# unanan/UNet_Nested4Tiny_Objects_Keypoints

Measured on AMD Instinct MI355X. Metric: images/sec (train step) UNet++ L=4 256x256, higher is better.
Workload: dtype f32

## Files before the change

include/unetpp_hip.h:

```cpp
#ifndef UNETPP_HIP_H
#define UNETPP_HIP_H

#include <stdint.h>

#ifdef __cplusplus
extern "C" {
#endif

#define UNETPP_ABI_VERSION 12
#define UNETPP_MAX_VIEWS 8

#define UNETPP_OK 0
#define UNETPP_EINVAL (-1)
#define UNETPP_ELAUNCH (-2)

typedef struct unetpp_view {
  float* ptr;
  int32_t C, c_off, c_len;
  int32_t Hs, Ws;
  int32_t sy, sx, oy, ox;
  const float* scale;
  const float* shift;
  const float* gate;
  int32_t relu;
// ... 135 lines not shown
                             int32_t W, int32_t C, float* dy, void* stream);

int64_t unetpp_bn_frozen_bwd_blocks(int64_t pixels, int32_t C);
int unetpp_bn_frozen_bwd(const float* d_act, const float* y, const float* scale, const float* shift,
                         const float* mean, const float* invstd, const float* d_pooled, const uint8_t* pool_idx,
                         int32_t N, int32_t H, int32_t W, int32_t C, float* dy, float* partial, void* stream);

int unetpp_head_fwd(const float* x, const float* weight, const float* bias, int32_t N, int32_t H, int32_t W,
                    int32_t C, int32_t n_cls, float p_drop, uint64_t seed, const uint8_t* mask, const uint64_t* seed_dev,
                    float* out_nchw, void* stream);
int64_t unetpp_head_bwd_blocks(int64_t pixels);
int unetpp_head_bwd(const float* d_out_nchw, const float* out_nchw, const float* x, const float* weight,
                    int32_t N, int32_t H, int32_t W, int32_t C, int32_t n_cls, float p_drop, uint64_t seed,
                    const uint8_t* mask, const uint64_t* seed_dev, float* dx, int32_t accumulate, int32_t gate_x, float* partial,
                    void* stream);
int unetpp_sum_partials(const float* partial, int64_t n_blocks, int64_t len, float* out, void* stream);

int unetpp_bilinear2x_fwd(const float* x, int32_t N, int32_t H, int32_t W, int32_t C, float* y, void* stream);
int unetpp_bilinear2x_bwd(const float* dy, int32_t N, int32_t H, int32_t W, int32_t C, float* dx, int32_t accumulate,
                          void* stream);

int64_t unetpp_focal_bce_blocks(int64_t n);
int unetpp_focal_bce(const float* pred, const float* target, int64_t n, int64_t rows, float gamma, float* grad,
                     float* partial, float* loss, void* stream);
#define UNETPP_MAX_HEADS 8
typedef struct unetpp_focal_heads {
  const float* pred[UNETPP_MAX_HEADS];
  float* grad[UNETPP_MAX_HEADS];
  int32_t n_heads, reserved;
} unetpp_focal_heads;
// ... 100 lines not shown
```

unet_nested4tiny_objects_keypoints_amd/_lib.py:

```python
from __future__ import annotations

import ctypes as C
import os
import subprocess

_PKG_DIR = os.path.dirname(os.path.abspath(__file__))
_REPO = os.path.dirname(_PKG_DIR)
LIB_PATH = os.environ.get("UNETPP_LIB", os.path.join(_PKG_DIR, "libunetpp_hip.so"))
CSRC = os.path.join(_PKG_DIR, "csrc")
INCLUDE = os.path.join(_REPO, "include")
SOURCES = ("gemm_pix.hip", "gemm_fast.hip", "gemm_pw.hip", "gemm_pw_bf16.hip", "gemm_wino.hip", "gemm_bf16.hip", "gemm_bf16_dma.hip", "wgrad_bf16.hip", "pointwise_bf16.hip", "keypoints.hip", "weight_image.hip", "wgrad.hip", "wgrad_fast.hip", "wgrad_dma.hip", "wgrad_pw.hip", "wgrad_wino.hip", "first_layer.hip", "pointwise.hip", "caller.hip", "optim.hip", "validate.hip")
HEADERS = ("common.h", "gemm_units.h", "wgrad_reduce.h", "lds_asm.h", "bf16_common.h", "dropout.h", "bn_fused.h",
           "wino_experiments.h", "dma_experiments.h", "heads_mean.h")
MAX_VIEWS = 8
ABI_VERSION = 12
EXTRA_FLAGS = {"gemm_wino.hip": ("-fno-slp-vectorize",), "wgrad_wino.hip": ("-fno-slp-vectorize",)}
GEMM_DIRECT = 1
GEMM_BF16 = 2


class View(C.Structure):
    _fields_ = [
        ("ptr", C.c_void_p),
        ("C", C.c_int32), ("c_off", C.c_int32), ("c_len", C.c_int32),
# ... 120 lines not shown
    "unetpp_pack_weight": (C.c_int, [_P, _P, _I32, _I32, _I32, _I64, _I64, _I64, _I64, _I64, _I64, _I32, _P]),
    "unetpp_bn_finalize": (C.c_int, [_P, _I64, _I32, _I64, _P, _P, _F, _F, _P, _P, _P, _P, _P, _P, _P]),
    "unetpp_bn_eval_coeffs": (C.c_int, [_P, _P, _P, _P, _F, _I32, _P, _P, _P]),
    "unetpp_affine_relu_pool": (C.c_int, [_P, _P, _P, _I32, _I32, _I32, _I32, _I32, _P, _P, _P, _P]),
    "unetpp_maxpool_bwd": (C.c_int, [_P, _P, _I32, _I32, _I32, _I32, _P, _P]),
    "unetpp_bn_bwd_blocks": (_I64, [_I64, _I32]),
    "unetpp_bn_bwd_reduce": (C.c_int, [_P, _P, _P, _P, _P, _P, _I64, _I32, _P, _P]),
    "unetpp_bn_bwd_finalize": (C.c_int, [_P, _I64, _I32, _P, _P, _P]),
    "unetpp_bn_bwd_apply": (C.c_int, [_P, _P, _P, _P, _P, _P, _P, _P, _P, _I64, _I32, _P, _P]),
    "unetpp_bn_bwd_pool_ok": (C.c_int, [_I32, _I32, _I32, _I32]),
    "unetpp_bn_bwd_reduce_pool": (C.c_int, [_P, _P, _P, _P, _P, _P, _P, _P, _I32, _I32, _I32, _I32, _P, _P]),
    "unetpp_bn_bwd_apply_pool": (C.c_int, [_P, _P, _P, _P, _P, _P, _P, _P, _P, _P, _P, _I32, _I32, _I32, _I32, _P, _P]),
    "unetpp_head_fwd": (C.c_int, [_P, _P, _P, _I32, _I32, _I32, _I32, _I32, _F, _U64, _P, _P, _P, _P]),
    "unetpp_head_bwd_blocks": (_I64, [_I64]),
    "unetpp_head_bwd": (C.c_int, [_P, _P, _P, _P, _I32, _I32, _I32, _I32, _I32, _F, _U64, _P, _P, _P, _I32, _I32, _P, _P]),
    "unetpp_sum_partials": (C.c_int, [_P, _I64, _I64, _P, _P]),
    "unetpp_focal_bce_blocks": (_I64, [_I64]),
    "unetpp_focal_bce": (C.c_int, [_P, _P, _I64, _I64, _F, _P, _P, _P, _P]),
    "unetpp_focal_bce_heads": (C.c_int, [C.POINTER(FocalHeads), _P, _I64, _I64, _F, _P, _P, _P]),
    "unetpp_heads_mean_fwd": (C.c_int, [C.POINTER(HeadsMean), _I32, _I32, _I32, _I32, _I32, _P, _P]),
    "unetpp_heads_mean_fwd_bf16": (C.c_int, [C.POINTER(HeadsMean), _I32, _I32, _I32, _I32, _I32, _P, _P]),
    "unetpp_bn_eval_coeffs_stats": (C.c_int, [_P, _P, _P, _P, _F, _I32, _P, _P, _P, _P, _P]),
    "unetpp_bn_frozen_bwd_blocks": (_I64, [_I64, _I32]),
    "unetpp_bn_frozen_bwd": (C.c_int, [_P, _P, _P, _P, _P, _P, _P, _P, _I32, _I32, _I32, _I32, _P, _P, _P]),
    "unetpp_bn_frozen_bwd_blocks_bf16": (_I64, [_I64, _I32]),
    "unetpp_bn_frozen_bwd_bf16": (C.c_int, [_P, _P, _P, _P, _P, _P, _P, _P, _I32, _I32, _I32, _I32, _P, _P, _P]),
    "unetpp_copy_jobs": (C.c_int, [_P, _I32, _I64, _P]),
    "unetpp_heatmap_workspace_bytes": (_I64, [_I32, _I32, _I32]),
    "unetpp_create_heatmap": (C.c_int, [_P, _I32, _I32, _I32, _I32, _F, _P, _P, _P]),
    "unetpp_bilinear2x_fwd": (C.c_int, [_P, _I32, _I32, _I32, _I32, _P, _P]),
# ... 111 lines not shown
```

unet_nested4tiny_objects_keypoints_amd/csrc/caller.hip:

```cpp
#include "common.h"

namespace unetpp {
namespace {

constexpr int kLossThreads = 256;
constexpr int kLossPerThread = 8;

__device__ __forceinline__ float focal_thread(const float* __restrict__ pred, float* __restrict__ grad,
                                              const float (&t)[kLossPerThread / 4][4], long base, long n, float gamma,
                                              float inv_rows, float scale) {
  const bool cube = gamma == 3.f;
  float sum = 0.f;
#pragma unroll
  for (int h = 0; h < kLossPerThread / 4; ++h) {
    const long i = base + 4 * h;
    if (i >= n) break;
    float p[4], g[4];
    const bool vec = (i + 4 <= n);
    if (vec) {
      const f32x4 pv = *reinterpret_cast<const f32x4*>(pred + i);
#pragma unroll
      for (int e = 0; e < 4; ++e) p[e] = pv[e];
    } else {
#pragma unroll
      for (int e = 0; e < 4; ++e) p[e] = (i + e < n) ? pred[i + e] : 0.f;
    }
#pragma unroll
    for (int e = 0; e < 4; ++e) {
      const float d = p[e] - t[h][e];
      const float err = (1.f - fabsf(d)) + 1e-20f;
      const float u = 1.f - err;
      const float lg = logf(err);
      const float ug1 = cube ? u * u : powf(u, gamma - 1.f);
      const float ug = ug1 * u;
      const float le = -ug * lg;
      const float dl_de = gamma * ug1 * lg - ug / err;
      const float sgn = (d > 0.f) ? 1.f : ((d < 0.f) ? -1.f : 0.f);
      g[e] = (-dl_de * sgn * inv_rows) * scale;
      if (i + e < n) sum += le;
    }
    if (grad != nullptr) {
      if (vec) {
        *reinterpret_cast<f32x4*>(grad + i) = f32x4{g[0], g[1], g[2], g[3]};
      } else {
#pragma unroll
        for (int e = 0; e < 4; ++e)
          if (i + e < n) grad[i + e] = g[e];
      }
    }
  }
  return sum;
}

// ... 231 lines not shown
```

unet_nested4tiny_objects_keypoints_amd/csrc/common.h:

```cpp
#pragma once
#include <hip/hip_runtime.h>
#include <stdint.h>

#include "unetpp_hip.h"

typedef float f32x16 __attribute__((ext_vector_type(16)));
typedef float f32x4 __attribute__((ext_vector_type(4)));

namespace unetpp {

constexpr int kBlockPixels = 256;
constexpr int kThreads = 256;
constexpr int kMaxHaloPixels = 340;

struct TileGeom {
  int log2tw, tiles_x, tiles_y;
};

inline TileGeom tile_geom(int H, int W) {
  int l = 3;
  while ((1 << l) < W && l < 5) ++l;
  TileGeom g;
  g.log2tw = l;
  const int TW = 1 << l, TH = kBlockPixels >> l;
// ... 7 lines not shown
  static_assert(OFF == 1 || OFF == 2 || OFF == 4 || OFF == 8 || OFF == 16, "xor_lane: 1, 2, 4, 8 or 16");
  const int i = __builtin_bit_cast(int, v);
  int r;
  if constexpr (OFF == 1) r = __builtin_amdgcn_mov_dpp(i, 0xB1, 0xF, 0xF, true);
  else if constexpr (OFF == 2) r = __builtin_amdgcn_mov_dpp(i, 0x4E, 0xF, 0xF, true);
  else r = __builtin_amdgcn_ds_swizzle(i, 0x1F | (OFF << 10));
  return __builtin_bit_cast(float, r);
}

__device__ __forceinline__ float row16_sum(float v) {
  v += xor_lane<1>(v);
  v += xor_lane<2>(v);
  v += __builtin_bit_cast(float, __builtin_amdgcn_mov_dpp(__builtin_bit_cast(int, v), 0x141, 0xF, 0xF, true));
  v += __builtin_bit_cast(float, __builtin_amdgcn_mov_dpp(__builtin_bit_cast(int, v), 0x140, 0xF, 0xF, true));
  return v;
}

inline int finish_log2_groups(int n_split) {
  int l = 0;
  while ((1 << l) < n_split && l < 4) ++l;
  return l;
}

inline bool view_ok(const unetpp_view& v, bool need_ptr = true) {
  if (need_ptr && v.ptr == nullptr) return false;
  if (v.C <= 0 || v.c_len <= 0 || v.c_off < 0 || v.c_off + v.c_len > v.C) return false;
  if (v.Hs <= 0 || v.Ws <= 0 || v.sy <= 0 || v.sx <= 0 || v.oy < 0 || v.ox < 0) return false;
  if ((v.scale == nullptr) != (v.shift == nullptr)) return false;
  return true;
}
// ... 127 lines not shown
```

unet_nested4tiny_objects_keypoints_amd/csrc/pointwise.hip:

```cpp
#include "common.h"
#include "lds_asm.h"
#include "dropout.h"
#include "heads_mean.h"

namespace unetpp {
namespace {

template <int VEC>
struct Pack;
template <>
struct Pack<4> {
  using T = f32x4;
};
template <>
struct Pack<1> {
  using T = float;
};
template <int VEC>
__device__ __forceinline__ float& lane_of(typename Pack<VEC>::T& v, int i) {
  if constexpr (VEC == 4)
    return reinterpret_cast<float*>(&v)[i];
  else
    return v;
}
// ... 1067 lines not shown
        f32x4 old = {0.f, 0.f, 0.f, 0.f};
        if (accumulate) old = *reinterpret_cast<const f32x4*>(dx + off);
#pragma unroll
        for (int q = 0; q < 4; ++q) {
          float v = sacc[q] * ms[q] + old[q];
          if (gate_x) v = (xv[q] > 0.f) ? v : 0.f;
          sacc[q] = v;
        }
        *reinterpret_cast<f32x4*>(dx + off) = sacc;
      }
      float* xd = &xs[pl * XS + 4 * gq];
#pragma unroll
      for (int q = 0; q < 4; ++q) xd[q] = xv[q] * ms[q];
    }
    __syncthreads();
#pragma unroll
    for (int q = 0; q < kMaxPairs; ++q) {
      if (pair0 + q * 128 < NW) {
        const int k = pair_k[q], c = pair_c[q];
        float sum = 0.f;
#pragma unroll 4
        for (int pl = 32 * half; pl < 32 * half + 32; ++pl) sum += dl[pl * kHeadMaxCls + k] * xs[pl * XS + c];
        wacc[q] += sum;
      }
    }
    if (tid < n_cls) {
      float sum = 0.f;
      for (int pl = 0; pl < 64; ++pl) sum += dl[pl * kHeadMaxCls + tid];
      bacc += sum;
    }
// ... 667 lines not shown
  if ((C & 3) == 0 && aligned16(x) && aligned16(dx)) {
    const size_t lds = (64 * (C + 1) + 64 * kHeadMaxCls + kHeadMaxCls * C + 2 * n_cls * C) * sizeof(float);
    note_kernel("head_bwd_vec");
    hipLaunchKernelGGL(head_bwd_vec_kernel, dim3(static_cast<unsigned>(unetpp_head_bwd_blocks(pixels))), dim3(kThreads),
                       lds, ST(stream), d_out_nchw, out_nchw, x, weight, pixels, H * W, C, n_cls, 1.0f / (1.0f - p_drop),
                       keep_threshold(p_drop), seed, mask, seed_dev, use_drop, dx, accumulate, gate_x, partial);
    return launch_status();
  }
  note_kernel("head_bwd");
  hipLaunchKernelGGL(head_bwd_kernel, dim3(static_cast<unsigned>(unetpp_head_bwd_blocks(pixels))), dim3(kThreads), 0,
                     ST(stream), d_out_nchw, out_nchw, x, weight, pixels, H * W, C, n_cls, 1.0f / (1.0f - p_drop),
                     keep_threshold(p_drop), seed, mask, seed_dev, use_drop, dx, accumulate, gate_x, partial);
  return launch_status();
}

extern "C" int unetpp_sum_partials(const float* partial, int64_t n_blocks, int64_t len, float* out, void* stream) {
  if (!partial || !out || n_blocks < 1 || len < 1) return UNETPP_EINVAL;
  hipLaunchKernelGGL(sum_partials_kernel, dim3(static_cast<unsigned>((len + 15) / 16)), dim3(1024), 0, ST(stream),
                     partial, n_blocks, len, out);
  return launch_status();
}

extern "C" int unetpp_bilinear2x_fwd(const float* x, int32_t N, int32_t H, int32_t W, int32_t C, float* y, void* stream) {
  if (!x || !y || N < 1 || H < 1 || W < 1 || C < 1) return UNETPP_EINVAL;
  const long items = static_cast<long>(N) * 4 * H * W * C;
  note_kernel("bilinear2x_fwd");
  hipLaunchKernelGGL(bilinear2x_fwd_kernel, dim3(grid_for(items)), dim3(kThreads), 0, ST(stream), x, N, H, W, C, y);
  return launch_status();
}

// ... 30 lines not shown
```

unet_nested4tiny_objects_keypoints_amd/engine.py:

```python
from __future__ import annotations

import os

from typing import Dict, List, Optional, Tuple

import torch

from . import ops
from .ops import V


USE_PACK_PLAN = os.environ.get("UNETPP_NO_PACK_PLAN") is None
USE_GROUPED_DGRAD = os.environ.get("UNETPP_NO_GROUPED_DGRAD") is None
USE_PLAN_COPIES = os.environ.get("UNETPP_NO_PLAN_COPIES") is None
_A1_MATERIALIZE_BYTES = int(float(os.environ.get("UNETPP_BF16_A1_MAX_MB", "80")) * (1 << 20))
_A1_MATERIALIZE_BYTES_F32 = int(float(os.environ.get("UNETPP_F32_A1_MAX_MB", "80")) * (1 << 20))


def _empty(n, like):
    return torch.empty(n, dtype=torch.float32, device=like.device)


def _packed(w, t, k, n, dstr, sstr, flip=False):
    dst = _empty(t * k * n, w)
# ... 198 lines not shown


def check_head(depth: int, head) -> int:
    if head is None:
        return depth - 1
    if isinstance(head, bool) or not isinstance(head, int) or not 1 <= head <= depth - 1:
        raise ValueError("head must be an int in 1..%d (or None for the last head), got %r" % (depth - 1, head))
    return head


def plan_phase(depth: int, head=None) -> str:
    head = check_head(depth, head)
    return "fwd" if head == depth - 1 else "fwd/%d" % head


def forward_impl(model, x, training: bool, save: bool, head: Optional[int] = None, ensemble: bool = False):
    _check_input(model, x)
    _PENDING_COUNTERS.clear()
    try:
        if not USE_PACK_PLAN:
            return _forward_impl(model, x, training, save, head, ensemble)
        plan = _plan_of(model)
        plan.begin(plan_phase(model.depth, head))
        ops.set_pack_plan(plan)
        try:
            return _forward_impl(model, x, training, save, head, ensemble)
        finally:
            ops.set_pack_plan(None)
    finally:
        flush_batch_counters()


def infer(model, x, head=None, ensemble: bool = False):
    top = check_head(model.depth, head)
    if model.training:
        raise RuntimeError("UNet_Nested.infer is the eval forward: call model.eval() first")
    pruned_to = getattr(model, "pruned_to", None)
    if pruned_to is not None and top > pruned_to:
        raise RuntimeError("this model holds a checkpoint pruned to head %d: the nodes head %d needs were never loaded"
                           % (pruned_to, top))
    if model.is_batchnorm:
# ... 3 lines not shown
                    raise RuntimeError("UNet_Nested.infer is the eval forward, but BatchNorm layer conv%d0.%s.1 is in training "
                                       "mode: call model.eval() (or .eval() on that layer) first" % (i, stage))
    with torch.no_grad():
        outs, _ = forward_impl(model, x, False, save=False, head=top, ensemble=bool(ensemble))
    return outs[0]


def _plan_of(model) -> "ops.PackPlan":
    plan = model.__dict__.get("_pack_plan")
    if plan is None:
        plan = ops.PackPlan()
        model.__dict__["_pack_plan"] = plan
    return plan


def _forward_impl(model, x, training: bool, save: bool, head: Optional[int] = None, ensemble: bool = False):
    b, _, h0, w0 = x.shape
    d = model.depth
    top = d - 1 if head is None else head
    adt = _activation_dtype(model)
    x_nhwc = ops.nchw_to_nhwc(x.detach().contiguous())
    X: Dict[Tuple[int, int], torch.Tensor] = {}
    pairs: Dict[Tuple[int, int], _PairRec] = {}
    ups: Dict[Tuple[int, int], _UpRec] = {}
    inp, h, w = x_nhwc, h0, w0
    for (i, j) in needed_nodes(d, top):
        if j == 0:
            with ops.region("X%d0.fwd" % i):
                r = _pair_fwd(getattr(model, "conv%d0" % i), [V(inp)], b, h, w, training, pool=(i < top), adt=adt,
                              stats=save)
            pairs[(i, 0)], X[(i, 0)] = r, r.out
# ... 3 lines not shown
            mod = getattr(model, "up_concat%d%d" % (i, j))
            hi, wi = h0 >> i, w0 >> i
            u = _up_fwd(mod.up, model.is_deconv, X[(i + 1, j - 1)], b, hi // 2, wi // 2, adt)
            ins = [V(u.up)] + [V(X[(i, jj)]) for jj in range(j)]
            r = _pair_fwd(mod.conv, ins, b, hi, wi, training, pool=False, adt=adt, stats=save)
            ups[(i, j)], pairs[(i, j)], X[(i, j)] = u, r, r.out
    p_drop, seeds, masks, seed_dev = _dropout_config(model, training)
    outs = []
    if head is not None and ensemble:
        finals = [getattr(model, "final_%d" % j) for j in range(1, head + 1)]
        o = torch.empty((b, model.n_classes, h0, w0), dtype=torch.float32, device=x.device)
        ops.heads_mean_fwd([X[(0, j)] for j in range(1, head + 1)],
                           [f.weight.detach().view(model.n_classes, -1) for f in finals],
                           [f.bias.detach() for f in finals], o)
        outs.append(o)
    for j in (range(1, d) if head is None else () if ensemble else (head,)):
        final = getattr(model, "final_%d" % j)
        o = torch.empty((b, model.n_classes, h0, w0), dtype=torch.float32, device=x.device)
        ops.head_fwd(X[(0, j)], final.weight.detach().view(model.n_classes, -1), final.bias.detach(), p_drop,
                     seeds[j - 1], None if masks is None else masks[j - 1], o, seed_dev=seed_dev)
        outs.append(o)
    if not save:
        return outs, None
    s = _Saved()
    s.x_nhwc, s.X, s.pairs, s.ups, s.outs = x_nhwc, X, pairs, ups, outs
    s.p_drop, s.seeds, s.masks, s.seed_dev = p_drop, seeds, masks, seed_dev
    s.shape = (b, h0, w0)
    return outs, s


class _GradBook:

    def __init__(self, X, depth, gate_keys, grouped=False):
        self.X = X
        self.buf: Dict[Tuple[int, int], torch.Tensor] = {}
        self.got: Dict[Tuple[int, int], int] = {}
        self.gate_keys = gate_keys
        self.gated = set()
        self.expected = {}
        for (i, j) in X:
            n = (1 if (i == 0 and j >= 1) else 0)
            consumers = max(0, (depth - 1 - i) - j)
# ... 147 lines not shown
    if not USE_PACK_PLAN:
        return _backward_impl(model, s, d_outs, want_input_grad, grad_sink)
    plan = _plan_of(model)
    plan.begin("bwd")
    ops.set_pack_plan(plan)
    try:
        return _backward_impl(model, s, d_outs, want_input_grad, grad_sink)
    finally:
        ops.set_pack_plan(None)


def _backward_impl(model, s: _Saved, d_outs, want_input_grad: bool, grad_sink=None):
    b, h0, w0 = s.shape
    d = model.depth
    grads: Dict[torch.nn.Parameter, torch.Tensor] = {}
    gate_keys = {k for k in s.X if k[1] >= 1 or not model.is_batchnorm}
    grouped = USE_GROUPED_DGRAD
    book = _GradBook(s.X, d, gate_keys, grouped)
    bf16 = s.X[(0, 0)].dtype == torch.bfloat16
    dy1s: Dict[Tuple[int, int], V] = {}
    seen = set()

    def flush():
        if grad_sink is not None and len(grads) > len(seen):
            fresh = [(p, g) for p, g in grads.items() if id(p) not in seen]
            seen.update(id(p) for p, _ in fresh)
            if fresh:
                grad_sink(fresh)

    for j in range(d - 1, 0, -1):
        head = getattr(model, "final_%d" % j)
        go = d_outs[j - 1]
        if go is None:
            go = torch.zeros_like(s.outs[j - 1])
        go = go.contiguous()
        dx, acc, gate = book.target((0, j), can_gate=True)
        dw, db = ops.head_bwd(go, s.outs[j - 1], s.X[(0, j)], head.weight.detach().view(model.n_classes, -1), s.p_drop,
                              s.seeds[j - 1], None if s.masks is None else s.masks[j - 1], dx, acc,
                              gate_x=gate is not None, seed_dev=s.seed_dev)
        if _ALLOC[0] is not None:
            gw, gb = _new_grad(head.weight), _new_grad(head.bias)
            gw.copy_(dw)
            gb.copy_(db)
            dw, db = gw, gb
        grads[head.weight], grads[head.bias] = dw, db
    flush()
    for j in range(d - 1, 0, -1):
        for i in range(d - 1 - j, -1, -1):
            mod = getattr(model, "up_concat%d%d" % (i, j))
            r, u = s.pairs[(i, j)], s.ups[(i, j)]
            d_out, pre_gated = book.take((i, j))
            d_up = torch.empty_like(u.up)
            targets = [V(d_up)]
            if grouped:
# ... 35 lines not shown
            pool_grad = (d_pooled, s.pairs[(i - 1, 0)].pool_idx)
        elif want_input_grad:
            if bf16 and s.x_nhwc.shape[3] > 4:
                raise NotImplementedError("bf16 storage: the input gradient needs at most 4 input channels")
            dx_in = torch.empty_like(s.x_nhwc)
            _pair_bwd(blk, r, d_out, [V(dx_in)], b, grads, pre_gated, pool_grad=mine, flush=flush)
        else:
            _pair_bwd(blk, r, d_out, None, b, grads, pre_gated, pool_grad=mine, flush=flush)
        flush()
    return grads, dx_in


class _UNetNestedFn(torch.autograd.Function):
    @staticmethod
    def forward(ctx, model, x, *params):
        outs, saved = forward_impl(model, x, model.training, save=True)
        if getattr(model, "_debug_keep_saved", False):
            model._debug_saved = saved
        ctx.model, ctx.saved = model, saved
        ctx.params = params
        return tuple(outs)

    @staticmethod
    @torch.autograd.function.once_differentiable
    def backward(ctx, *d_outs):
        model, saved = ctx.model, ctx.saved
        if saved is None:
            raise RuntimeError("UNet_Nested (HIP): backward called twice on the same forward")
        ctx.saved = None
        sink = getattr(model, "_grad_sink", None)
        _ALLOC[0] = getattr(model, "_grad_alloc", None)
# ... 22 lines not shown
```

unet_nested4tiny_objects_keypoints_amd/graph.py:

```python
from __future__ import annotations

import collections
import copy
import ctypes
import os
import warnings
from typing import Optional

import torch

from .step import loss_and_backward

_HIP_NODE_TYPES = {0: "kernel", 1: "memcpy", 2: "memset", 3: "host", 4: "graph", 5: "empty", 6: "wait_event",
                   7: "event_record", 8: "ext_sem_signal", 9: "ext_sem_wait", 10: "mem_alloc", 11: "mem_free",
                   12: "memcpy_from_symbol", 13: "memcpy_to_symbol"}


def _loaded_hip_runtime():
    path = None
    with open("/proc/self/maps") as f:
        for ln in f:
            if "libamdhip64.so" in ln:
                path = ln.split()[-1]
                break
    if path is None:
        raise RuntimeError("no libamdhip64.so is loaded in this process (is torch's HIP runtime initialised?)")
# ... 121 lines not shown
                            v.copy_(old[k])
                        else:
                            v.zero_()
                    elif k in old:
                        st[k] = copy.deepcopy(old[k])
                    elif isinstance(v, (int, float)):
                        st[k] = type(v)(0)
        if self._plan is not None:
            self._plan.invalidate()

    def _new_seed(self):
        self._seed.fill_(int(torch.randint(0, 2 ** 62, (1,)).item()))

    def _body(self, with_optimizer: bool):
        self.optimizer.zero_grad(set_to_none=True)
        outputs = self.model(self._x)
        avgloss = loss_and_backward(self.criterion, outputs, self._t)
        if with_optimizer:
            self.optimizer.step()
        return outputs, avgloss

    def __call__(self, inputs: torch.Tensor, target: torch.Tensor):
        if inputs.shape != self._x.shape or inputs.dtype != self._x.dtype or inputs.device != self._x.device:
            raise ValueError("GraphedTrainStep was captured for inputs %s %s on %s, got %s %s on %s" % (
                tuple(self._x.shape), self._x.dtype, self._x.device, tuple(inputs.shape), inputs.dtype, inputs.device))
        if target.shape != self._t.shape or target.dtype != self._t.dtype or target.device != self._t.device:
            raise ValueError("GraphedTrainStep was captured for targets %s %s, got %s %s" % (
                tuple(self._t.shape), self._t.dtype, tuple(target.shape), target.dtype))
        if not self.model.training:
            raise RuntimeError("the captured graph is a training step; the model is in eval mode")
        if [p.data_ptr() for p in self.model.parameters()] != self._param_ptrs:
            raise RuntimeError("the model's parameters moved (.to() / load with assign) since the graph was captured: "
# ... 19 lines not shown
```

unet_nested4tiny_objects_keypoints_amd/ops.py:

```python
from __future__ import annotations

import ctypes as C
import functools
import os
from dataclasses import dataclass
from typing import Optional, Sequence

import torch

from . import _lib
from ._lib import MAX_VIEWS, GemmDesc, PackJob, View, WeightSrc, WgradDesc, check


def _stream():
    return C.c_void_p(torch.cuda.current_stream().cuda_stream)


class LaunchTimer:

    def __init__(self):
        self.launches = []
        self.regions = []
        self.want_launches = True
        self.want_regions = True
# ... 633 lines not shown
    lib = _lib.lib()
    n, h, w, c = x.shape
    n_cls = weight.shape[0]
    blocks = int(lib.unetpp_head_bwd_blocks(n * h * w))
    ln = n_cls * c + n_cls
    partial = torch.empty(blocks * ln, dtype=torch.float32, device=x.device)
    sums = torch.empty(ln, dtype=torch.float32, device=x.device)
    st = _stream()
    fn = lib.unetpp_head_bwd_bf16 if _is_bf16(x) else lib.unetpp_head_bwd
    check(fn(_ptr(d_out), _ptr(out), _ptr(x), _ptr(weight), n, h, w, c, n_cls, float(p_drop), C.c_uint64(seed), _ptr(mask),
             _ptr(seed_dev), _ptr(dx), int(accumulate), int(gate_x), _ptr(partial), st), "unetpp_head_bwd")
    check(lib.unetpp_sum_partials(_ptr(partial), blocks, ln, _ptr(sums), st), "unetpp_sum_partials")
    return sums[:n_cls * c].view(n_cls, c, 1, 1), sums[n_cls * c:]


def bilinear2x_fwd(x, y):
    n, h, w, c = x.shape
    if _is_bf16(x):
        check(_lib.lib().unetpp_bilinear2x_fwd_bf16(_ptr(x), n, h, w, c, _ptr(y), _stream()), "unetpp_bilinear2x_fwd_bf16")
        return
    check(_lib.lib().unetpp_bilinear2x_fwd(_ptr(x), n, h, w, c, _ptr(y), _stream()), "unetpp_bilinear2x_fwd")


def bilinear2x_bwd(dy, dx, accumulate, gate=None):
    n, h, w, c = dx.shape
    if _is_bf16(dx):
        check(_lib.lib().unetpp_bilinear2x_bwd_bf16(_ptr(dy), n, h, w, c, _ptr(dx), int(accumulate), _ptr(gate), _stream()),
              "unetpp_bilinear2x_bwd_bf16")
        return
    if gate is not None:
# ... 235 lines not shown
```

unet_nested4tiny_objects_keypoints_amd/step.py:

```python
from __future__ import annotations

import os

import torch

_FUSED_HEAD_LOSS = os.environ.get("UNETPP_NO_FUSED_HEAD_LOSS") is None


def loss_and_backward(criterion, outputs, target):
    if isinstance(outputs, tuple):
        fused = getattr(criterion, "mean_over_heads", None)
        if _FUSED_HEAD_LOSS and fused is not None and torch.is_grad_enabled() and all(o.requires_grad for o in outputs):
            got = fused(outputs, target)
            if got is not None:
                avgloss, grads = got
                torch.autograd.backward(list(outputs), grads)
                return avgloss
        avgloss = 0
        for output in outputs:
            avgloss = avgloss + criterion(output, target)
        avgloss = 1.0 * avgloss / len(outputs)
    else:
        avgloss = criterion(outputs, target)
    avgloss.backward()
    return avgloss


def train_step(model, optimizer, criterion, inputs, target):
    optimizer.zero_grad()
    outputs = model(inputs)
    avgloss = loss_and_backward(criterion, outputs, target)
    optimizer.step()
    return outputs, avgloss
```

Measured before the change: 1712.

## Fuse deep-supervision head forward, focal loss gradient and head backward into one kernel

Adds a head_train kernel that computes the 1x1 head logits, sigmoid output, focal BCE gradient, input gradient and weight/bias partials in a single pass, called during the forward when the criterion is the package focal loss. The later head backward then reuses the precomputed grads instead of running its own kernels. This removes separate head_fwd, focal_bce and head_bwd launches and the extra reads and writes of features and outputs. The cost is more engine coupling, since a HeadLoss object is passed through model state, plus an extra loss-only evaluation pass and a fallback path when its conditions are not met.

```diff
diff --git a/include/unetpp_hip.h b/include/unetpp_hip.h
--- a/include/unetpp_hip.h
+++ b/include/unetpp_hip.h
@@ -173,6 +173,10 @@
                     int32_t N, int32_t H, int32_t W, int32_t C, int32_t n_cls, float p_drop, uint64_t seed,
                     const uint8_t* mask, const uint64_t* seed_dev, float* dx, int32_t accumulate, int32_t gate_x, float* partial,
                     void* stream);
+int unetpp_head_train(const float* x, const float* weight, const float* bias, const float* target, int32_t N, int32_t H,
+                      int32_t W, int32_t C, int32_t n_cls, float p_drop, uint64_t seed, const uint8_t* mask,
+                      const uint64_t* seed_dev, float gamma, float inv_rows, float scale, float* out_nchw, float* dx,
+                      int32_t accumulate, int32_t gate_x, float* partial, void* stream);
 int unetpp_sum_partials(const float* partial, int64_t n_blocks, int64_t len, float* out, void* stream);
 
 int unetpp_bilinear2x_fwd(const float* x, int32_t N, int32_t H, int32_t W, int32_t C, float* y, void* stream);
diff --git a/unet_nested4tiny_objects_keypoints_amd/_lib.py b/unet_nested4tiny_objects_keypoints_amd/_lib.py
--- a/unet_nested4tiny_objects_keypoints_amd/_lib.py
+++ b/unet_nested4tiny_objects_keypoints_amd/_lib.py
@@ -158,6 +158,8 @@
     "unetpp_head_fwd": (C.c_int, [_P, _P, _P, _I32, _I32, _I32, _I32, _I32, _F, _U64, _P, _P, _P, _P]),
     "unetpp_head_bwd_blocks": (_I64, [_I64]),
     "unetpp_head_bwd": (C.c_int, [_P, _P, _P, _P, _I32, _I32, _I32, _I32, _I32, _F, _U64, _P, _P, _P, _I32, _I32, _P, _P]),
+    "unetpp_head_train": (C.c_int, [_P, _P, _P, _P, _I32, _I32, _I32, _I32, _I32, _F, _U64, _P, _P, _F, _F, _F, _P, _P,
+                                    _I32, _I32, _P, _P]),
     "unetpp_sum_partials": (C.c_int, [_P, _I64, _I64, _P, _P]),
     "unetpp_focal_bce_blocks": (_I64, [_I64]),
     "unetpp_focal_bce": (C.c_int, [_P, _P, _I64, _I64, _F, _P, _P, _P, _P]),
diff --git a/unet_nested4tiny_objects_keypoints_amd/csrc/caller.hip b/unet_nested4tiny_objects_keypoints_amd/csrc/caller.hip
--- a/unet_nested4tiny_objects_keypoints_amd/csrc/caller.hip
+++ b/unet_nested4tiny_objects_keypoints_amd/csrc/caller.hip
@@ -27,16 +27,9 @@
     }
 #pragma unroll
     for (int e = 0; e < 4; ++e) {
-      const float d = p[e] - t[h][e];
-      const float err = (1.f - fabsf(d)) + 1e-20f;
-      const float u = 1.f - err;
-      const float lg = logf(err);
-      const float ug1 = cube ? u * u : powf(u, gamma - 1.f);
-      const float ug = ug1 * u;
+      float ug, lg;
+      g[e] = focal_bce_grad(p[e], t[h][e], gamma, cube, inv_rows, scale, ug, lg);
       const float le = -ug * lg;
-      const float dl_de = gamma * ug1 * lg - ug / err;
-      const float sgn = (d > 0.f) ? 1.f : ((d < 0.f) ? -1.f : 0.f);
-      g[e] = (-dl_de * sgn * inv_rows) * scale;
       if (i + e < n) sum += le;
     }
     if (grad != nullptr) {
diff --git a/unet_nested4tiny_objects_keypoints_amd/csrc/common.h b/unet_nested4tiny_objects_keypoints_amd/csrc/common.h
--- a/unet_nested4tiny_objects_keypoints_amd/csrc/common.h
+++ b/unet_nested4tiny_objects_keypoints_amd/csrc/common.h
@@ -45,6 +45,22 @@
   v += __builtin_bit_cast(float, __builtin_amdgcn_mov_dpp(__builtin_bit_cast(int, v), 0x141, 0xF, 0xF, true));
   v += __builtin_bit_cast(float, __builtin_amdgcn_mov_dpp(__builtin_bit_cast(int, v), 0x140, 0xF, 0xF, true));
   return v;
+}
+
+__device__ __forceinline__ float focal_bce_grad(float p, float t, float gamma, bool cube, float inv_rows, float scale,
+                                                float& ug, float& lg) {
+  const float d = p - t;
+  const float err = (1.f - fabsf(d)) + 1e-20f;
+  const float u = 1.f - err;
+  lg = logf(err);
+  const float ug1 = cube ? u * u : powf(u, gamma - 1.f);
+  ug = ug1 * u;
+  const float sgn = (d > 0.f) ? 1.f : ((d < 0.f) ? -1.f : 0.f);
+  {
+#pragma clang fp contract(off)
+    const float dl_de = gamma * ug1 * lg - ug / err;
+    return (-dl_de * sgn * inv_rows) * scale;
+  }
 }
 
 inline int finish_log2_groups(int n_split) {
diff --git a/unet_nested4tiny_objects_keypoints_amd/csrc/pointwise.hip b/unet_nested4tiny_objects_keypoints_amd/csrc/pointwise.hip
--- a/unet_nested4tiny_objects_keypoints_amd/csrc/pointwise.hip
+++ b/unet_nested4tiny_objects_keypoints_amd/csrc/pointwise.hip
@@ -1105,6 +1105,182 @@
       for (int q = 0; q < 4; ++q) xd[q] = xv[q] * ms[q];
     }
     __syncthreads();
+#pragma unroll
+    for (int q = 0; q < kMaxPairs; ++q) {
+      if (pair0 + q * 128 < NW) {
+        const int k = pair_k[q], c = pair_c[q];
+        float sum = 0.f;
+#pragma unroll 4
+        for (int pl = 32 * half; pl < 32 * half + 32; ++pl) sum += dl[pl * kHeadMaxCls + k] * xs[pl * XS + c];
+        wacc[q] += sum;
+      }
+    }
+    if (tid < n_cls) {
+      float sum = 0.f;
+      for (int pl = 0; pl < 64; ++pl) sum += dl[pl * kHeadMaxCls + tid];
+      bacc += sum;
+    }
+  }
+  __syncthreads();
+#pragma unroll
+  for (int q = 0; q < kMaxPairs; ++q) {
+    const int idx = pair0 + q * 128;
+    if (idx < NW) scratch[half * NW + idx] = wacc[q];
+  }
+  __syncthreads();
+  float* dst = partial + static_cast<long>(blockIdx.x) * (NW + n_cls);
+  for (int i = tid; i < NW; i += kThreads) dst[i] = scratch[i] + scratch[NW + i];
+  if (tid < n_cls) dst[NW + tid] = bacc;
+}
+
+template <int LOG2G, int DROP, int PCLS>
+__global__ __launch_bounds__(kThreads, ((4 << LOG2G) / 4 + 4 * PCLS >= 48) ? 2 : 4) void head_train_pow2_kernel(const float* __restrict__ x,
+                                                                   const float* __restrict__ weight,
+                                                                   const float* __restrict__ bias,
+                                                                   const float* __restrict__ target, unsigned pixels,
+                                                                   unsigned HW, int n_cls, float keep_scale, uint32_t thr16,
+                                                                   uint64_t seed, const uint8_t* __restrict__ mask,
+                                                                   const uint64_t* __restrict__ seed_dev, float gamma,
+                                                                   float inv_rows, float scale, float* __restrict__ out,
+                                                                   float* __restrict__ dx, int accumulate, int gate_x,
+                                                                   float* __restrict__ partial) {
+  if (seed_dev != nullptr) seed += *seed_dev;
+  extern __shared__ __attribute__((aligned(16))) float hsm[];
+  constexpr int G = 1 << LOG2G, C = 4 * G, XS = C + 1;
+  static_assert(G >= PCLS && (64 * G) % kThreads == 0, "head_train_pow2_kernel: C / 4 >= padded classes");
+  constexpr int ITEMS = 64 * G / kThreads;
+  constexpr int kDup = G / PCLS;
+  constexpr int kElems = PCLS / 4;
+  const int NW = n_cls * C;
+  float* xs = hsm;
+  float* dl = xs + 64 * XS;
+  float* scratch = dl + 64 * kHeadMaxCls;
+  const int tid = threadIdx.x;
+  const int gq = tid & (G - 1);
+  const bool cube = gamma == 3.f;
+  f32x4 wq[PCLS];
+#pragma unroll
+  for (int k = 0; k < PCLS; ++k)
+    wq[k] = (k < n_cls) ? *reinterpret_cast<const f32x4*>(weight + k * C + 4 * gq) : f32x4{0.f, 0.f, 0.f, 0.f};
+  constexpr int kMaxPairs = (PCLS * C + 127) / 128;
+  float wacc[kMaxPairs];
+  int pair_k[kMaxPairs], pair_c[kMaxPairs];
+  const int pair0 = tid & 127, half = tid >> 7;
+#pragma unroll
+  for (int q = 0; q < kMaxPairs; ++q) {
+    wacc[q] = 0.f;
+    const int idx = pair0 + q * 128;
+    pair_k[q] = idx >> (LOG2G + 2);
+    pair_c[q] = idx & (C - 1);
+  }
+  float bacc = 0.f;
+  for (int i = tid; i < 64 * kHeadMaxCls; i += kThreads) dl[i] = 0.f;
+  const unsigned n_tiles = (pixels + 63) / 64;
+  for (unsigned tile = blockIdx.x; tile < n_tiles; tile += gridDim.x) {
+    const unsigned p0 = tile * 64;
+    __syncthreads();
+    unsigned eo[kElems];
+    float tv[kElems];
+#pragma unroll
+    for (int e = 0; e < kElems; ++e) {
+      const int it = tid + e * kThreads, pl = it & 63, k = it >> 6;
+      const unsigned p = p0 + pl;
+      eo[e] = ~0u;
+      tv[e] = 0.f;
+      if (k < n_cls && p < pixels) {
+        const unsigned n = p / HW, hw = p - n * HW;
+        eo[e] = (n * n_cls + k) * HW + hw;
+        tv[e] = target[eo[e]];
+      }
+    }
+    f32x4 xv[ITEMS];
+    uint32_t m4[ITEMS];
+#pragma unroll
+    for (int u = 0; u < ITEMS; ++u) {
+      const unsigned p = p0 + ((tid + u * kThreads) >> LOG2G);
+      const unsigned off = (p << (LOG2G + 2)) + 4 * gq;
+      xv[u] = (p < pixels) ? *reinterpret_cast<const f32x4*>(x + off) : f32x4{0.f, 0.f, 0.f, 0.f};
+      if constexpr (DROP == 2) m4[u] = (p < pixels) ? *reinterpret_cast<const uint32_t*>(mask + off) : 0u;
+    }
+    uint32_t kept = 0, pos = 0;
+#pragma unroll
+    for (int u = 0; u < ITEMS; ++u) {
+      const int pl = (tid + u * kThreads) >> LOG2G;
+      uint32_t k4 = 0xfu;
+      if constexpr (DROP == 1) {
+        const uint64_t bits = keep_bits(seed, p0 + pl, G, gq);
+        k4 = 0;
+#pragma unroll
+        for (int q = 0; q < 4; ++q) k4 |= keep_one(bits, q, thr16) ? (1u << q) : 0u;
+      } else if constexpr (DROP == 2) {
+        k4 = 0;
+#pragma unroll
+        for (int q = 0; q < 4; ++q) k4 |= ((m4[u] >> (8 * q)) & 0xffu) != 0 ? (1u << q) : 0u;
+      }
+      kept |= k4 << (4 * u);
+      f32x4 v = xv[u];
+      float* xd = &xs[pl * XS + 4 * gq];
+#pragma unroll
+      for (int q = 0; q < 4; ++q) {
+        if (gate_x) pos |= (xv[u][q] > 0.f) ? (1u << (4 * u + q)) : 0u;
+        if constexpr (DROP != 0) {
+          const bool keep = (k4 >> q) & 1u;
+          v[q] = keep ? xv[u][q] * keep_scale : 0.f;
+          xd[q] = xv[u][q] * (keep ? keep_scale : 0.f);
+        } else {
+          xd[q] = xv[u][q];
+        }
+      }
+      int cls;
+      const float logit = head_pixel_logit<LOG2G, PCLS>(v, wq, gq, cls);
+      if (cls < n_cls && (gq & (kDup - 1)) == 0) dl[pl * kHeadMaxCls + cls] = logit;
+    }
+    __syncthreads();
+#pragma unroll
+    for (int e = 0; e < kElems; ++e) {
+      const int it = tid + e * kThreads, pl = it & 63, k = it >> 6;
+      if (k < n_cls) {
+        float dlv = 0.f;
+        if (eo[e] != ~0u) {
+          const float pr = 1.0f / (1.0f + __expf(-(dl[pl * kHeadMaxCls + k] + bias[k])));
+          out[eo[e]] = pr;
+          float ug, lg;
+          const float g = focal_bce_grad(pr, tv[e], gamma, cube, inv_rows, scale, ug, lg);
+          dlv = g * pr * (1.f - pr);
+        }
+        dl[pl * kHeadMaxCls + k] = dlv;
+      }
+    }
+    __syncthreads();
+#pragma unroll
+    for (int u = 0; u < ITEMS; ++u) {
+      const int pl = (tid + u * kThreads) >> LOG2G;
+      const unsigned p = p0 + pl;
+      if (p < pixels) {
+        const unsigned off = (p << (LOG2G + 2)) + 4 * gq;
+        float ms[4] = {1.f, 1.f, 1.f, 1.f};
+        if constexpr (DROP != 0) {
+#pragma unroll
+          for (int q = 0; q < 4; ++q) ms[q] = ((kept >> (4 * u + q)) & 1u) ? keep_scale : 0.f;
+        }
+        f32x4 sacc = {0.f, 0.f, 0.f, 0.f};
+#pragma unroll
+        for (int k = 0; k < PCLS; ++k) {
+          const float dk = dl[pl * kHeadMaxCls + k];
+#pragma unroll
+          for (int q = 0; q < 4; ++q) sacc[q] += wq[k][q] * dk;
+        }
+        f32x4 old = {0.f, 0.f, 0.f, 0.f};
+        if (accumulate) old = *reinterpret_cast<const f32x4*>(dx + off);
+#pragma unroll
+        for (int q = 0; q < 4; ++q) {
+          float v = sacc[q] * ms[q] + old[q];
+          if (gate_x) v = ((pos >> (4 * u + q)) & 1u) ? v : 0.f;
+          sacc[q] = v;
+        }
+        *reinterpret_cast<f32x4*>(dx + off) = sacc;
+      }
+    }
 #pragma unroll
     for (int q = 0; q < kMaxPairs; ++q) {
       if (pair0 + q * 128 < NW) {
@@ -1802,6 +1978,55 @@
   return launch_status();
 }
 
+extern "C" int unetpp_head_train(const float* x, const float* weight, const float* bias, const float* target, int32_t N,
+                                 int32_t H, int32_t W, int32_t C, int32_t n_cls, float p_drop, uint64_t seed,
+                                 const uint8_t* mask, const uint64_t* seed_dev, float gamma, float inv_rows, float scale,
+                                 float* out_nchw, float* dx, int32_t accumulate, int32_t gate_x, float* partial,
+                                 void* stream) {
+  if (!x || !weight || !bias || !target || !out_nchw || !dx || !partial || !head_args_ok(N, H, W, C, n_cls, p_drop))
+    return UNETPP_EINVAL;
+  const long pixels = static_cast<long>(N) * H * W;
+  const int g4 = C >> 2;
+  const int pcls = n_cls <= 4 ? 4 : 8;
+  if (!((C & 3) == 0 && aligned16(x) && aligned16(dx) && aligned16(weight) && (g4 & (g4 - 1)) == 0 && g4 >= pcls && g4 <= 32 &&
+        pixels * C < 0x7fffffffL && (mask == nullptr || (reinterpret_cast<uintptr_t>(mask) & 3) == 0)))
+    return 1;
+  const size_t lds = (64 * (C + 1) + 64 * kHeadMaxCls + 2 * n_cls * C) * sizeof(float);
+  const dim3 grid(static_cast<unsigned>(unetpp_head_bwd_blocks(pixels)));
+  const int drop = !(p_drop > 0.f) ? 0 : (mask == nullptr ? 1 : 2);
+#define UNETPP_HEAD_TRAIN_P(L, D, PC)                                                                                 \
+  do {                                                                                                              \
+    note_kernel("head_train_pow2<" #L "," #D "," #PC ">");                                                          \
+    hipLaunchKernelGGL((head_train_pow2_kernel<L, D, PC>), grid, dim3(kThreads), lds, ST(stream), x, weight, bias,   \
+                       target, static_cast<unsigned>(pixels), static_cast<unsigned>(H * W), n_cls,                   \
+                       1.0f / (1.0f - p_drop), keep_threshold(p_drop), seed, mask, seed_dev, gamma, inv_rows, scale,  \
+                       out_nchw, dx, accumulate, gate_x, partial);                                                  \
+  } while (0)
+#define UNETPP_HEAD_TRAIN(L, PC)                         \
+  do {                                                   \
+    if (drop == 0) UNETPP_HEAD_TRAIN_P(L, 0, PC);        \
+    else if (drop == 1) UNETPP_HEAD_TRAIN_P(L, 1, PC);   \
+    else UNETPP_HEAD_TRAIN_P(L, 2, PC);                  \
+  } while (0)
+  if (pcls == 4) {
+    switch (g4) {
+      case 4: UNETPP_HEAD_TRAIN(2, 4); break;
+      case 8: UNETPP_HEAD_TRAIN(3, 4); break;
+      case 16: UNETPP_HEAD_TRAIN(4, 4); break;
+      default: UNETPP_HEAD_TRAIN(5, 4); break;
+    }
+  } else {
+    switch (g4) {
+      case 8: UNETPP_HEAD_TRAIN(3, 8); break;
+      case 16: UNETPP_HEAD_TRAIN(4, 8); break;
+      default: UNETPP_HEAD_TRAIN(5, 8); break;
+    }
+  }
+#undef UNETPP_HEAD_TRAIN
+#undef UNETPP_HEAD_TRAIN_P
+  return launch_status();
+}
+
 extern "C" int unetpp_sum_partials(const float* partial, int64_t n_blocks, int64_t len, float* out, void* stream) {
   if (!partial || !out || n_blocks < 1 || len < 1) return UNETPP_EINVAL;
   hipLaunchKernelGGL(sum_partials_kernel, dim3(static_cast<unsigned>((len + 15) / 16)), dim3(1024), 0, ST(stream),
diff --git a/unet_nested4tiny_objects_keypoints_amd/engine.py b/unet_nested4tiny_objects_keypoints_amd/engine.py
--- a/unet_nested4tiny_objects_keypoints_amd/engine.py
+++ b/unet_nested4tiny_objects_keypoints_amd/engine.py
@@ -236,17 +236,18 @@
     return "fwd" if head == depth - 1 else "fwd/%d" % head
 
 
-def forward_impl(model, x, training: bool, save: bool, head: Optional[int] = None, ensemble: bool = False):
+def forward_impl(model, x, training: bool, save: bool, head: Optional[int] = None, ensemble: bool = False,
+                 head_loss: Optional["HeadLoss"] = None):
     _check_input(model, x)
     _PENDING_COUNTERS.clear()
     try:
         if not USE_PACK_PLAN:
-            return _forward_impl(model, x, training, save, head, ensemble)
+            return _forward_impl(model, x, training, save, head, ensemble, head_loss)
         plan = _plan_of(model)
         plan.begin(plan_phase(model.depth, head))
         ops.set_pack_plan(plan)
         try:
-            return _forward_impl(model, x, training, save, head, ensemble)
+            return _forward_impl(model, x, training, save, head, ensemble, head_loss)
         finally:
             ops.set_pack_plan(None)
     finally:
@@ -280,7 +281,20 @@
     return plan
 
 
-def _forward_impl(model, x, training: bool, save: bool, head: Optional[int] = None, ensemble: bool = False):
+class HeadLoss:
+    __slots__ = ("target", "rows", "gamma", "taken")
+
+    def __init__(self, target, rows, gamma):
+        self.target, self.rows, self.gamma, self.taken = target, rows, gamma, False
+
+
+def _new_book(model, X):
+    gate_keys = {k for k in X if k[1] >= 1 or not model.is_batchnorm}
+    return _GradBook(X, model.depth, gate_keys, USE_GROUPED_DGRAD)
+
+
+def _forward_impl(model, x, training: bool, save: bool, head: Optional[int] = None, ensemble: bool = False,
+                  head_loss: Optional[HeadLoss] = None):
     b, _, h0, w0 = x.shape
     d = model.depth
     top = d - 1 if head is None else head
@@ -314,7 +328,26 @@
                            [f.weight.detach().view(model.n_classes, -1) for f in finals],
                            [f.bias.detach() for f in finals], o)
         outs.append(o)
-    for j in (range(1, d) if head is None else () if ensemble else (head,)):
+    book, head_grads = None, None
+    if (head_loss is not None and save and training and head is None and adt == torch.float32
+            and all(ops.head_train_takes(X[(0, j)].shape[3], model.n_classes, X[(0, j)].numel(),
+                                         getattr(model, "final_%d" % j).weight, None if masks is None else masks[j - 1])
+                    for j in range(1, d))):
+        book, head_grads = _new_book(model, X), {}
+        for j in range(1, d):
+            final = getattr(model, "final_%d" % j)
+            o = torch.empty((b, model.n_classes, h0, w0), dtype=torch.float32, device=x.device)
+            dx, acc, gate = book.target((0, j), can_gate=True)
+            got = ops.head_train(X[(0, j)], final.weight.detach().view(model.n_classes, -1), final.bias.detach(),
+                                 head_loss.target, head_loss.rows, head_loss.gamma, d - 1, p_drop, seeds[j - 1],
+                                 None if masks is None else masks[j - 1], o, dx, acc, gate_x=gate is not None,
+                                 seed_dev=seed_dev)
+            if got is None:
+                raise RuntimeError("unetpp_head_train did not take a shape that ops.head_train_takes accepts")
+            head_grads[j] = got
+            outs.append(o)
+        head_loss.taken = True
+    for j in (() if book is not None else range(1, d) if head is None else () if ensemble else (head,)):
         final = getattr(model, "final_%d" % j)
         o = torch.empty((b, model.n_classes, h0, w0), dtype=torch.float32, device=x.device)
         ops.head_fwd(X[(0, j)], final.weight.detach().view(model.n_classes, -1), final.bias.detach(), p_drop,
@@ -326,6 +359,7 @@
     s.x_nhwc, s.X, s.pairs, s.ups, s.outs = x_nhwc, X, pairs, ups, outs
     s.p_drop, s.seeds, s.masks, s.seed_dev = p_drop, seeds, masks, seed_dev
     s.shape = (b, h0, w0)
+    s.book, s.head_grads = book, head_grads
     return outs, s
 
 
@@ -503,9 +537,8 @@
     b, h0, w0 = s.shape
     d = model.depth
     grads: Dict[torch.nn.Parameter, torch.Tensor] = {}
-    gate_keys = {k for k in s.X if k[1] >= 1 or not model.is_batchnorm}
     grouped = USE_GROUPED_DGRAD
-    book = _GradBook(s.X, d, gate_keys, grouped)
+    book = s.book if s.book is not None else _new_book(model, s.X)
     bf16 = s.X[(0, 0)].dtype == torch.bfloat16
     dy1s: Dict[Tuple[int, int], V] = {}
     seen = set()
@@ -519,14 +552,17 @@
 
     for j in range(d - 1, 0, -1):
         head = getattr(model, "final_%d" % j)
-        go = d_outs[j - 1]
-        if go is None:
-            go = torch.zeros_like(s.outs[j - 1])
-        go = go.contiguous()
-        dx, acc, gate = book.target((0, j), can_gate=True)
-        dw, db = ops.head_bwd(go, s.outs[j - 1], s.X[(0, j)], head.weight.detach().view(model.n_classes, -1), s.p_drop,
-                              s.seeds[j - 1], None if s.masks is None else s.masks[j - 1], dx, acc,
-                              gate_x=gate is not None, seed_dev=s.seed_dev)
+        if s.head_grads is not None:
+            dw, db = s.head_grads[j]
+        else:
+            go = d_outs[j - 1]
+            if go is None:
+                go = torch.zeros_like(s.outs[j - 1])
+            go = go.contiguous()
+            dx, acc, gate = book.target((0, j), can_gate=True)
+            dw, db = ops.head_bwd(go, s.outs[j - 1], s.X[(0, j)], head.weight.detach().view(model.n_classes, -1), s.p_drop,
+                                  s.seeds[j - 1], None if s.masks is None else s.masks[j - 1], dx, acc,
+                                  gate_x=gate is not None, seed_dev=s.seed_dev)
         if _ALLOC[0] is not None:
             gw, gb = _new_grad(head.weight), _new_grad(head.bias)
             gw.copy_(dw)
@@ -592,7 +628,7 @@
 class _UNetNestedFn(torch.autograd.Function):
     @staticmethod
     def forward(ctx, model, x, *params):
-        outs, saved = forward_impl(model, x, model.training, save=True)
+        outs, saved = forward_impl(model, x, model.training, save=True, head_loss=model.__dict__.get("_head_loss"))
         if getattr(model, "_debug_keep_saved", False):
             model._debug_saved = saved
         ctx.model, ctx.saved = model, saved
diff --git a/unet_nested4tiny_objects_keypoints_amd/graph.py b/unet_nested4tiny_objects_keypoints_amd/graph.py
--- a/unet_nested4tiny_objects_keypoints_amd/graph.py
+++ b/unet_nested4tiny_objects_keypoints_amd/graph.py
@@ -9,7 +9,7 @@
 
 import torch
 
-from .step import loss_and_backward
+from .step import forward_loss_backward
 
 _HIP_NODE_TYPES = {0: "kernel", 1: "memcpy", 2: "memset", 3: "host", 4: "graph", 5: "empty", 6: "wait_event",
                    7: "event_record", 8: "ext_sem_signal", 9: "ext_sem_wait", 10: "mem_alloc", 11: "mem_free",
@@ -161,8 +161,7 @@
 
     def _body(self, with_optimizer: bool):
         self.optimizer.zero_grad(set_to_none=True)
-        outputs = self.model(self._x)
-        avgloss = loss_and_backward(self.criterion, outputs, self._t)
+        outputs, avgloss = forward_loss_backward(self.model, self.criterion, self._x, self._t)
         if with_optimizer:
             self.optimizer.step()
         return outputs, avgloss
diff --git a/unet_nested4tiny_objects_keypoints_amd/ops.py b/unet_nested4tiny_objects_keypoints_amd/ops.py
--- a/unet_nested4tiny_objects_keypoints_amd/ops.py
+++ b/unet_nested4tiny_objects_keypoints_amd/ops.py
@@ -671,6 +671,39 @@
     return sums[:n_cls * c].view(n_cls, c, 1, 1), sums[n_cls * c:]
 
 
+def head_train_takes(c, n_cls, elements, *tensors):
+    g4 = c >> 2
+    pcls = 4 if n_cls <= 4 else 8
+    return (c == 4 * g4 and g4 & (g4 - 1) == 0 and pcls <= g4 <= 32 and 1 <= n_cls <= 8 and elements < 0x7fffffff
+            and all(t is None or t.data_ptr() % 16 == 0 for t in tensors))
+
+
+def head_train(x, weight, bias, target, rows, gamma, heads, p_drop, seed, mask, out_nchw, dx, accumulate, gate_x=False,
+               seed_dev=None):
+    lib = _lib.lib()
+    n, h, w, c = x.shape
+    n_cls = weight.shape[0]
+    _need(x, "head features")
+    _need(target, "target")
+    if tuple(target.shape) != (n, n_cls, h, w) or tuple(_need(out_nchw, "output").shape) != (n, n_cls, h, w):
+        raise ValueError("target and output must be [N, n_cls, H, W]")
+    blocks = int(lib.unetpp_head_bwd_blocks(n * h * w))
+    ln = n_cls * c + n_cls
+    partial = torch.empty(blocks * ln, dtype=torch.float32, device=x.device)
+    inv_rows = C.c_float(1.0 / C.c_float(float(rows)).value)
+    scale = C.c_float(1.0 / C.c_float(float(heads)).value)
+    st = _stream()
+    status = lib.unetpp_head_train(_ptr(x), _ptr(weight), _ptr(bias), _ptr(target), n, h, w, c, n_cls, float(p_drop),
+                                   C.c_uint64(seed), _ptr(mask), _ptr(seed_dev), float(gamma), inv_rows, scale,
+                                   _ptr(out_nchw), _ptr(dx), int(accumulate), int(gate_x), _ptr(partial), st)
+    if status == 1:
+        return None
+    check(status, "unetpp_head_train")
+    sums = torch.empty(ln, dtype=torch.float32, device=x.device)
+    check(lib.unetpp_sum_partials(_ptr(partial), blocks, ln, _ptr(sums), st), "unetpp_sum_partials")
+    return sums[:n_cls * c].view(n_cls, c, 1, 1), sums[n_cls * c:]
+
+
 def bilinear2x_fwd(x, y):
     n, h, w, c = x.shape
     if _is_bf16(x):
diff --git a/unet_nested4tiny_objects_keypoints_amd/step.py b/unet_nested4tiny_objects_keypoints_amd/step.py
--- a/unet_nested4tiny_objects_keypoints_amd/step.py
+++ b/unet_nested4tiny_objects_keypoints_amd/step.py
@@ -7,9 +7,19 @@
 _FUSED_HEAD_LOSS = os.environ.get("UNETPP_NO_FUSED_HEAD_LOSS") is None
 
 
+def _fused_heads_enabled():
+    return os.environ.get("UNETPP_NO_FUSED_HEADS") is None
+
+
+def _is_package_focal(criterion):
+    from .losses import FocalLoss_BCE_2d
+    return (isinstance(criterion, FocalLoss_BCE_2d) and type(criterion).forward is FocalLoss_BCE_2d.forward
+            and not criterion._forward_hooks and not criterion._forward_pre_hooks)
+
+
 def loss_and_backward(criterion, outputs, target):
     if isinstance(outputs, tuple):
-        fused = getattr(criterion, "mean_over_heads", None)
+        fused = getattr(criterion, "mean_over_heads", None) if _is_package_focal(criterion) else None
         if _FUSED_HEAD_LOSS and fused is not None and torch.is_grad_enabled() and all(o.requires_grad for o in outputs):
             got = fused(outputs, target)
             if got is not None:
@@ -26,9 +36,44 @@
     return avgloss
 
 
+def _head_loss_for(model, criterion, inputs, target):
+    from . import _lib, engine
+    from .unet import UNet_Nested
+    if not (_FUSED_HEAD_LOSS and _fused_heads_enabled() and torch.is_grad_enabled() and _is_package_focal(criterion)):
+        return None
+    if not (isinstance(model, UNet_Nested) and model.training and model.is_ds and 2 <= model.depth - 1 <= _lib.MAX_HEADS
+            and getattr(model, "activation_dtype", torch.float32) == torch.float32):
+        return None
+    if not (torch.is_tensor(inputs) and inputs.dim() == 4 and torch.is_tensor(target) and target.is_cuda
+            and target.dtype == torch.float32 and target.is_contiguous() and not target.requires_grad
+            and target.device == inputs.device
+            and tuple(target.shape) == (inputs.shape[0], model.n_classes, inputs.shape[2], inputs.shape[3])):
+        return None
+    rows = target.numel() if criterion.size_average else target.shape[0] * target.shape[1]
+    return engine.HeadLoss(target, rows, float(criterion.gamma))
+
+
+def forward_loss_backward(model, criterion, inputs, target):
+    head_loss = _head_loss_for(model, criterion, inputs, target)
+    if head_loss is None:
+        outputs = model(inputs)
+        return outputs, loss_and_backward(criterion, outputs, target)
+    model.__dict__["_head_loss"] = head_loss
+    try:
+        outputs = model(inputs)
+    finally:
+        del model.__dict__["_head_loss"]
+    if not head_loss.taken:
+        return outputs, loss_and_backward(criterion, outputs, target)
+    from . import ops
+    heads = [o.detach() for o in outputs]
+    loss, _ = ops.focal_bce_heads(heads, target, head_loss.rows, head_loss.gamma, want_grad=False)
+    torch.autograd.backward(list(outputs), heads)
+    return outputs, loss[0]
+
+
 def train_step(model, optimizer, criterion, inputs, target):
     optimizer.zero_grad()
-    outputs = model(inputs)
-    avgloss = loss_and_backward(criterion, outputs, target)
+    outputs, avgloss = forward_loss_backward(model, criterion, inputs, target)
     optimizer.step()
     return outputs, avgloss
```

Result: no change. 1727, median of 6 (+0.9%).
